# IvanPopov/video-flow-ml

Hardware: AMD Instinct MI355X
Metric: flow-fields/sec @1080p seq5 MOF_sintel (higher is better)
Workload: dtype mixed (per-layer MFMA count, f32 accumulate): {"corr": 1, "update_block.encoder.convf1": 1, "update_block.encoder.convf2": 1, "update_block.gru.convq1.iter": "2a", "update_block.gru.convzr1.iter": 1, "update_block.gru.convzr2.iter": 1, "update_block.mask.0": 1, "update_block.mask.2": 1, "update_bloc

## Files before the change

include/vfml.h:

```cpp
#ifndef VFML_H
#define VFML_H
#include <stddef.h>
#include <stdint.h>

#ifdef __cplusplus
extern "C" {
#endif

#define VFML_ABI_VERSION 25

enum {
  VFML_EPI_NONE = 0,
  VFML_EPI_RELU = 1,
  VFML_EPI_TANH = 2,
  VFML_EPI_SIGMOID = 3,
  VFML_EPI_TANH_RELU = 4,
  VFML_EPI_GRU_ZR = 5,
  VFML_EPI_GRU_Q = 6,
  VFML_EPI_ADD_AUX = 7,
};

enum { VFML_FMT_F32 = 0, VFML_FMT_S16 = 1,
       VFML_FMT_F16 = 2 };

typedef struct vfml_conv_desc {
  const float* in0; int32_t c0; int32_t ld0;
  const float* in1; int32_t c1; int32_t ld1;
  int32_t n, h, w;
  const float* weight;
  const float* bias;
  int32_t cout, kh, kw, stride, pad_h, pad_w;
  float* out; int32_t ldo;
  int32_t epilogue; int32_t split; float out_scale;
  const float* aux0; int32_t ld_aux0;
  const float* aux1; int32_t ld_aux1;
  const float* addend; int32_t ld_addend;
  float* out_t; int32_t ld_out_t;
  int32_t flags;
  double* stats_part;
  float* ksplit_ws;
  const void* proj_hi; const void* proj_lo; int32_t proj_n; int32_t proj_kp; float proj_scale;
  float* proj_out; int32_t ld_proj;
  const float* const* addend_ind;
} vfml_conv_desc;

enum { VFML_STATS_ROWS_F32 = 128, VFML_STATS_ROWS_S16 = 32 };
enum { VFML_CONV_SWAP_CROSS = 1,
       VFML_CONV_MFMA2 = 2, VFML_CONV_MFMA1 = 4, VFML_CONV_MFMA2A = 8,
       VFML_CONV_PER_TAP = 16 };

int vfml_conv2d(const vfml_conv_desc* d, void* stream);

int vfml_conv2d_split(const vfml_conv_desc* d, const void* w_hi, const void* w_lo, int kp, float w_scale,
                      int in_fmt, int out_fmt, int aux_fmt, int k_order, void* stream);
enum { VFML_KORDER_TAP = 0, VFML_KORDER_CBLOCK = 1, VFML_KORDER_CBLOCK64 = 2 };

int vfml_to_s16(const float* src, int64_t rows, int c, int ld_src, float* dst, int ld_dst, float scale, void* stream);

int vfml_split_f16(const float* src, int64_t rows, int k, int ld, float scale, void* hi, void* lo, int kp,
                   void* stream);

int vfml_softmax_rows_s16(const float* x, int64_t rows, int cols, int64_t ld_in, float* out, int64_t ld_out, float scale,
                          void* stream);

int vfml_softmax_rows_f16(const float* x, int64_t rows, int cols, int64_t ld_in, void* out, int64_t ld_out, float scale,
                          void* stream);

int vfml_transpose_to_s16(const float* src, int rows, int c, int ld, float scale, float* dst, int64_t ld_dst, void* stream);

int vfml_add_to_s16(const float* x, int64_t ldx, const float* aux, int64_t ld_aux, float* out, int64_t ld_out, int64_t rows,
                    int c, float scale, void* stream);

int vfml_transpose_split_f16(const float* src, int rows, int c, int ld, float scale, void* hi, void* lo, int kp,
                             void* stream);

int vfml_frames_to_nhwc4(const void* src, int kind, int n, int H, int W,
                         float scale, float shift, float* dst, void* stream);

int64_t vfml_instnorm_workspace_bytes(int n, int hw, int c);
int vfml_instnorm_stats(const float* x, int n, int hw, int c, float eps,
                        float* stats, void* workspace, void* stream);
int vfml_instnorm_apply(const float* x, const float* stats, const float* res,
                        const float* res_stats, int n, int hw, int c, float* out, int out_fmt, void* stream);

int vfml_avgpool2x2(const float* x, int n, int h, int w, int c, float* out, void* stream);

int vfml_corr_lookup(const float* const* pyr, const int32_t* hl, const int32_t* wl,
                     const int32_t* ld, int levels, int radius, int nmaps, int q_per_map,
                     const float* coords, int ld_coords, float* out, int ld_out, int out_fmt, int vol_fmt, int vol_tile,
                     void* stream);
#define VFML_VOL_F16_LEVELS(m) (0x100 | (m))

int vfml_corr_lookup_indirect(const float* const* table, const int32_t* hl, const int32_t* wl, const int32_t* ld,
                              int levels, int radius, int nmaps, int q_per_map, const float* coords, int ld_coords,
                              float* out, int ld_out, int out_fmt, int vol_fmt, int vol_tile, void* stream);
int vfml_corr_lookup_indirect_bidir(const float* const* table, const int32_t* hl, const int32_t* wl, const int32_t* ld,
                                    int levels, int radius, int nmaps, int q_per_map, const float* coords, int ld_coords,
                                    int dir_coords, float* out, int ld_out, int dir_out, int dir_tab, int out_fmt, int vol_fmt,
                                    int vol_tile, void* stream);
int vfml_ptr_table_set(void* table, const void* const* ptrs, int n, void* stream);

int vfml_flow_rows7(const float* flow, int n, int h, int w, float* rows, void* stream);

int vfml_conv3x3_c64(const float* in, int ld_in, int n, int h, int w, const void* w_hi, const void* w_lo, int kp, float w_scale,
                     const float* bias, float* out, int ldo, double* stats_part, void* stream);

int vfml_flow_half(const float* flow, int n, int h, int w, const void* w1_hi, int kp1, float w1_scale, const float* b1,
                   const void* w2_hi, int kp2, float w2_scale, const float* b2, float* out, int ld_out, void* stream);

int vfml_tapsum3x3(const float* t, int ld_t, const float* bias, int n, int h, int w, float* out, int parts, int64_t part_stride,
                   void* stream);
int vfml_tapsum3x3_update(const float* t, int ld_t, const float* bias, int n, int h, int w, int parts, int64_t part_stride,
                          float* coords1, float* flow_a, int ld_a, float* flow_b, int ld_b, int fmt_b, void* stream);

int vfml_coords_update(float* coords1, const float* delta, int n, int h, int w,
                       float* flow_a, int ld_a, float* flow_b, int ld_b, int fmt_b, void* stream);
int vfml_coords_init(float* coords1, int n, int h, int w, void* stream);

int vfml_convex_upsample(const float* coords1, int ch, const float* mask, int ld_mask,
                         int h, int w, float* out, void* stream);

int64_t vfml_instnorm_finalize_workspace_bytes(int chunks, int c);
int vfml_instnorm_finalize(const double* part, int n, int chunks, int c, int hw, float eps, float* stats,
                           void* workspace, int64_t workspace_bytes, void* stream);

int vfml_stem7x7s2_chunks(int h, int w);
int vfml_stem7x7s2(const float* frames, int n, int h, int w, const void* w_hi, const void* w_lo, float w_scale,
                   const float* bias, float* out, double* stats_part, void* stream);

int vfml_flow_lod(const float* flow, int h, int w, float* out, void* stream);

enum { VFML_ENCODE_GAMEDEV = 0, VFML_ENCODE_RG8 = 1, VFML_ENCODE_RGB8 = 2 };
int vfml_flow_encode(const float* flow, int h, int w, int mode, float width, float height, float scale,
                     float clamp, float two_clamp, unsigned char* out, void* stream);

enum { VFML_TAA_SIMPLE = 0, VFML_TAA_BILINEAR = 1, VFML_TAA_BILATERAL = 2 };
enum { VFML_PIX_U8 = 0, VFML_PIX_F32 = 1, VFML_PIX_F64 = 2 };
int vfml_taa_blend(const void* current, int cur_type, const float* flow, const void* history, int hist_type,
                   void* out, int out_type, int h, int w, int mode, double alpha, double sigma_color, void* stream);

int vfml_flow_quality_map(const unsigned char* frame1, const unsigned char* frame2, const float* flow, int fh, int fw,
                          int h, int w, float threshold, unsigned char* out, void* stream);

#define VFML_CORRECT_RECORD 16
size_t vfml_flow_correct_workspace_bytes(int h, int w);
int vfml_flow_correct(const unsigned char* frame1, const unsigned char* frame2, const float* flow, const float* lod,
                      int lh, int lw, int h, int w, const double* twiddles, double good_threshold,
                      double fine_threshold, double region_radius, double template_radius, double search_radius,
                      float* out_flow, int* counts, double* records, int64_t record_capacity, void* workspace,
                      size_t workspace_bytes, void* stream);

enum { VFML_COLORIZE_HSV = 0, VFML_COLORIZE_WHEEL = 1 };
int vfml_flow_colorize(const float* flow, int h, int w, int mode, void* workspace, unsigned char* out, void* stream);

enum { VFML_COMPOSE_SIDE_BY_SIDE = 0, VFML_COMPOSE_STACKED = 1, VFML_COMPOSE_GRID_2X2 = 2 };
enum { VFML_COMPOSE_BGR = 1, VFML_COMPOSE_BOTTOM_UP = 2 };
int vfml_compose_frame(const void* const* tiles, const int* tile_types, int h, int w, int layout, int flags,
                       int64_t row_stride, unsigned char* out, void* stream);

const char* vfml_last_error(void);
int vfml_abi_version(void);

#ifdef __cplusplus
}
#endif
#endif
```

video-flow-ml_amd/vfml/csrc/flow_ops.hip:

```cpp
#include <stdlib.h>
#include "vfml_common.h"

namespace {

constexpr int MAX_LEVELS = 6;
constexpr int MAX_MAPS = 8;
constexpr int MAX_RADIUS = 4;
constexpr int PATCH = 2 * MAX_RADIUS + 2;
#ifndef VFML_LOOKUP_WAVES
#define VFML_LOOKUP_WAVES 4
#endif
constexpr int LOOKUP_WAVES = VFML_LOOKUP_WAVES;
constexpr int FIXED_LEVELS = 4;
static_assert(FIXED_LEVELS == 4, "corr_lookup_fixed_kernel selects among four levels");

struct LookupArgs {
  const float* pyr[MAX_MAPS][MAX_LEVELS];
  const float* const* table;
  int hl[MAX_LEVELS], wl[MAX_LEVELS], ld[MAX_LEVELS];
  int levels, radius, nq, q_per_map;
  const float* coords; int ld_coords;
  float* out; int ld_out;
  int out16;
  int vol16;
  int tws, ths;
  int qw;
  int dir_maps, dir_coords, dir_out;
  int dir_tab;
};

__device__ __forceinline__ void lookup_rows(const LookupArgs& a, int q, int& map, int64_t& crow, int64_t& orow) {
  const int dir = a.dir_maps && map >= a.dir_maps;
  const int64_t qd = q - (dir ? a.dir_maps * a.q_per_map : 0);
  if (dir) map += a.dir_tab - a.dir_maps;
  crow = qd * a.ld_coords + (dir ? a.dir_coords : 0);
  orow = qd * a.ld_out + (dir ? a.dir_out : 0);
}

__device__ __forceinline__ int tiled_at(int y, int x, int w, int tws, int ths) {
  const int tpr = (w + (1 << tws) - 1) >> tws;
  return ((((y >> ths) * tpr + (x >> tws)) << (tws + ths)) + ((y & ((1 << ths) - 1)) << tws) + (x & ((1 << tws) - 1)));
}

__device__ __forceinline__ float bilinear4(float nw, float ne, float sw, float se, float wx0, float fx, float wy0, float fy) {
  float v = ne * (fx * wy0);
  v = __builtin_fmaf(nw, wx0 * wy0, v);
  v = __builtin_fmaf(sw, wx0 * fy, v);
  v = __builtin_fmaf(se, fx * fy, v);
  return v;
}

__global__ __launch_bounds__(64 * LOOKUP_WAVES) void corr_lookup_kernel(const LookupArgs a) {
  __shared__ float patch[LOOKUP_WAVES][MAX_LEVELS][PATCH * PATCH];
  __shared__ float frac[LOOKUP_WAVES][MAX_LEVELS][2];
  const int lane = threadIdx.x & 63;
  const int wv = threadIdx.x >> 6;
  const int q = blockIdx.x * LOOKUP_WAVES + wv;
  const bool live = q < a.nq;
  int map = live ? q / a.q_per_map : 0;
  const int qq = q - map * a.q_per_map;
  const int side = 2 * a.radius + 2;
  const int win = 2 * a.radius + 1;
  const int psz = side * side;
  int64_t crow = 0, orow = 0;
  if (live) lookup_rows(a, q, map, crow, orow);
  if (live) {
    const float cx = a.coords[crow + 0];
    const float cy = a.coords[crow + 1];
    const int total = a.levels * psz;
    const int qrow = (a.tws | a.ths) ? tiled_at(qq / a.qw, qq % a.qw, a.qw, a.tws, a.ths) : qq;
    for (int e = lane; e < total; e += 64) {
      const int l = e / psz;
      const int idx = e - l * psz;
      const int py = idx / side, px = idx - py * side;
      const float inv = 1.0f / (float)(1 << l);
      const float x = cx * inv, y = cy * inv;
      const float fx0 = floorf(x), fy0 = floorf(y);
      const int x0 = (int)fminf(fmaxf(fx0, -65536.f), 65536.f) - a.radius;
      const int y0 = (int)fminf(fmaxf(fy0, -65536.f), 65536.f) - a.radius;
      const int xx = x0 + px, yy = y0 + py;
      float v = 0.f;
      if (xx >= 0 && xx < a.wl[l] && yy >= 0 && yy < a.hl[l])
        v = (a.table ? a.table[map * a.levels + l] : a.pyr[map][l])[(int64_t)qrow * a.ld[l] + tiled_at(yy, xx, a.wl[l], a.tws, a.ths)];
      patch[wv][l][idx] = v;
      if (idx == 0) {
        frac[wv][l][0] = x - fx0;
        frac[wv][l][1] = y - fy0;
      }
    }
  }
  __syncthreads();
  if (!live) return;
  const int nout = a.levels * win * win;
  float* o = a.out + orow;
  const int nwrite = a.out16 ? (nout + 7) & ~7 : nout;
  for (int c = lane; c < nwrite; c += 64) {
    if (c >= nout) {
      _Float16* u = reinterpret_cast<_Float16*>(o + (c & ~7));
      u[c & 7] = (_Float16)0.f;
      u[8 + (c & 7)] = (_Float16)0.f;
      continue;
    }
    const int l = c / (win * win);
    const int rem = c - l * win * win;
    const int i = rem / win, j = rem - i * win;
    const float fx = frac[wv][l][0], fy = frac[wv][l][1];
    const float* p = &patch[wv][l][j * side + i];
    const float wx0 = 1.f - fx, wy0 = 1.f - fy;
    const float v = bilinear4(p[0], p[1], p[side], p[side + 1], wx0, fx, wy0, fy);
    if (a.out16) {
      vfml_h16x2 hh, ll;
      vfml_split2(v, 0.f, hh, ll);
      _Float16* u = reinterpret_cast<_Float16*>(o + (c & ~7));
      u[c & 7] = hh[0];
      u[8 + (c & 7)] = ll[0];
    } else {
      o[c] = v;
    }
  }
}

__device__ __forceinline__ float bilinear4w(float nw, float ne, float sw, float se, float w00, float w10, float w01, float w11) {
  float v = ne * w10;
  v = __builtin_fmaf(nw, w00, v);
  v = __builtin_fmaf(sw, w01, v);
  v = __builtin_fmaf(se, w11, v);
  return v;
}

__device__ __forceinline__ void wave_lds_sync() {
  __builtin_amdgcn_fence(__ATOMIC_RELEASE, "workgroup");
  __builtin_amdgcn_wave_barrier();
  __builtin_amdgcn_fence(__ATOMIC_ACQUIRE, "workgroup");
}

template <int R, bool OUT16, int V16 = 0>
__global__ __launch_bounds__(64 * LOOKUP_WAVES) void corr_lookup_fixed_kernel(const LookupArgs a) {
  constexpr int SIDE = 2 * R + 2, PSZ = SIDE * SIDE, WIN = 2 * R + 1, WW = WIN * WIN;
  constexpr int NOUTPAD = (FIXED_LEVELS * WW + 7) & ~7;
  static_assert(PSZ <= 128 && FIXED_LEVELS * WIN <= 64 && NOUTPAD / 8 <= 64, "one wave: at most two gather passes per level");
  __shared__ float patch[LOOKUP_WAVES][FIXED_LEVELS][PSZ];
  __shared__ __attribute__((aligned(16))) float outs[LOOKUP_WAVES][NOUTPAD];
  const int lane = threadIdx.x & 63;
  const int wv = __builtin_amdgcn_readfirstlane(threadIdx.x >> 6);
  const int q = blockIdx.x * LOOKUP_WAVES + wv;
  if (q >= a.nq) return;
  int map = __builtin_amdgcn_readfirstlane(q / a.q_per_map);
  const int qq = q - map * a.q_per_map;
  const int qrow = __builtin_amdgcn_readfirstlane((a.tws | a.ths) ? tiled_at(qq / a.qw, qq % a.qw, a.qw, a.tws, a.ths) : qq);
  int64_t crow, orow;
  lookup_rows(a, q, map, crow, orow);
  const float cx = a.coords[crow + 0];
  const float cy = a.coords[crow + 1];
  const int pyA = lane / SIDE, pxA = lane - pyA * SIDE;
  const int pyB = (lane + 64) / SIDE, pxB = (lane + 64) - pyB * SIDE;
  const bool inB = lane + 64 < PSZ;
  const float* pl[FIXED_LEVELS];
  if (a.table) {
#pragma unroll
    for (int l = 0; l < FIXED_LEVELS; ++l) pl[l] = a.table[map * a.levels + (l < a.levels ? l : 0)];
  } else {
#pragma unroll
    for (int l = 0; l < FIXED_LEVELS; ++l) pl[l] = a.pyr[map][l < a.levels ? l : 0];
  }
  float va[FIXED_LEVELS], vb[FIXED_LEVELS];
  bool oka[FIXED_LEVELS], okb[FIXED_LEVELS];
#pragma unroll
  for (int l = 0; l < FIXED_LEVELS; ++l) {
    const bool have = l < a.levels;
    const int ll = have ? l : 0;
    const bool v16 = (V16 >> l) & 1;
    const int ES = v16 ? 2 : 4;
    const char* base = reinterpret_cast<const char*>(pl[l]) + (int64_t)qrow * a.ld[ll] * ES;
    const int wl = a.wl[ll], hl = a.hl[ll];
    const float inv = __builtin_bit_cast(float, (127 - l) << 23);
    const float x = cx * inv, y = cy * inv;
    const int x0 = (int)fminf(fmaxf(floorf(x), -65536.f), 65536.f) - R;
    const int y0 = (int)fminf(fmaxf(floorf(y), -65536.f), 65536.f) - R;
    auto texel = [&](int px, int py, bool in, float& out, bool& ok) {
      const int xx = x0 + px, yy = y0 + py;
      ok = have && in && xx >= 0 && xx < wl && yy >= 0 && yy < hl;
      const int at = tiled_at(min(max(yy, 0), hl - 1), min(max(xx, 0), wl - 1), wl, a.tws, a.ths);
      if (v16) out = (float)((const __attribute__((address_space(1))) _Float16*)base)[at];
      else out = ((const __attribute__((address_space(1))) float*)base)[at];
    };
    texel(pxA, pyA, true, va[l], oka[l]);
    if constexpr (PSZ > 64) texel(pxB, pyB, inB, vb[l], okb[l]);
    else { vb[l] = 0.f; okb[l] = false; }
  }
#pragma unroll
  for (int l = 0; l < FIXED_LEVELS; ++l) {
    va[l] = oka[l] ? va[l] : 0.f;
    vb[l] = okb[l] ? vb[l] : 0.f;
  }
#pragma unroll
  for (int l = 0; l < FIXED_LEVELS; ++l) {
    if (l < a.levels) {
      if (PSZ > 64 || lane < PSZ) patch[wv][l][lane] = va[l];
      if constexpr (PSZ > 64) if (inB) patch[wv][l][lane + 64] = vb[l];
    }
  }
  const int nout = a.levels * WW;
  const int nunits = (nout + 7) >> 3;
  if (lane >= 56 && nout + (lane - 56) < nunits * 8) outs[wv][nout + (lane - 56)] = 0.f;
  wave_lds_sync();
  if (lane < a.levels * WIN) {
    const int l = lane / WIN, i = lane - l * WIN;
    const float inv = __builtin_bit_cast(float, (127 - l) << 23);
    const float x = cx * inv, y = cy * inv;
    const float fx = x - floorf(x), fy = y - floorf(y);
    const float wx0 = 1.f - fx, wy0 = 1.f - fy;
    const float w00 = wx0 * wy0, w10 = fx * wy0, w01 = wx0 * fy, w11 = fx * fy;
    const float* p = &patch[wv][l][i];
    float* o = &outs[wv][l * WW + i * WIN];
    float nw = p[0], ne = p[1];
#pragma unroll
    for (int j = 0; j < WIN; ++j) {
      const float sw = p[(j + 1) * SIDE], se = p[(j + 1) * SIDE + 1];
      o[j] = bilinear4w(nw, ne, sw, se, w00, w10, w01, w11);
      nw = sw; ne = se;
    }
  }
  wave_lds_sync();
  if (lane < nunits) {
    float* o = a.out + orow + lane * 8;
    const f32x4 v0 = *reinterpret_cast<const f32x4*>(&outs[wv][lane * 8]);
    const f32x4 v1 = *reinterpret_cast<const f32x4*>(&outs[wv][lane * 8 + 4]);
    if (OUT16) {
      vfml_h16x2 h0, h1, h2, h3, l0, l1, l2, l3;
      vfml_split2(v0[0], v0[1], h0, l0);
      vfml_split2(v0[2], v0[3], h1, l1);
      vfml_split2(v1[0], v1[1], h2, l2);
      vfml_split2(v1[2], v1[3], h3, l3);
      uint4 hv, lv;
      hv.x = __builtin_bit_cast(unsigned, h0); hv.y = __builtin_bit_cast(unsigned, h1);
      hv.z = __builtin_bit_cast(unsigned, h2); hv.w = __builtin_bit_cast(unsigned, h3);
      lv.x = __builtin_bit_cast(unsigned, l0); lv.y = __builtin_bit_cast(unsigned, l1);
      lv.z = __builtin_bit_cast(unsigned, l2); lv.w = __builtin_bit_cast(unsigned, l3);
      *reinterpret_cast<uint4*>(o) = hv;
      *reinterpret_cast<uint4*>(o + 4) = lv;
    } else {
#pragma unroll
      for (int h = 0; h < 2; ++h) {
        const int c = lane * 8 + 4 * h;
        const f32x4 w = h ? v1 : v0;
        if (c + 3 < nout && (((uintptr_t)(o + 4 * h)) & 15u) == 0) {
          *reinterpret_cast<f32x4*>(o + 4 * h) = w;
        } else {
#pragma unroll
          for (int k = 0; k < 4; ++k)
            if (c + k < nout) o[4 * h + k] = w[k];
        }
      }
    }
  }
}

__global__ void coords_init_kernel(f32x4* __restrict__ coords, int h, int w, int64_t total) {
  for (int64_t p = (int64_t)blockIdx.x * blockDim.x + threadIdx.x; p < total; p += (int64_t)gridDim.x * blockDim.x) {
    const int x = (int)(p % w);
    const int y = (int)((p / w) % h);
    f32x4 v = {(float)x, (float)y, (float)x, (float)y};
    coords[p] = v;
  }
}

__global__ void flow_rows7_kernel(const f32x4* __restrict__ flow, int w, int64_t total, char* __restrict__ rows) {
  for (int64_t i = (int64_t)blockIdx.x * blockDim.x + threadIdx.x; i < total * 4; i += (int64_t)gridDim.x * blockDim.x) {
    const int64_t p = i >> 2;
    const int u = (int)(i & 3);
    const int x = (int)(p % w);
    f32x4 t0 = {0.f, 0.f, 0.f, 0.f}, t1 = {0.f, 0.f, 0.f, 0.f};
    const int x0 = x + 2 * u - 3, x1 = x0 + 1;
    if (x0 >= 0 && x0 < w) t0 = flow[p + 2 * u - 3];
    if (u < 3 && x1 >= 0 && x1 < w) t1 = flow[p + 2 * u - 2];
    vfml_h16x2 h[4], l[4];
    vfml_split2(t0[0], t0[1], h[0], l[0]);
    vfml_split2(t0[2], t0[3], h[1], l[1]);
    vfml_split2(t1[0], t1[1], h[2], l[2]);
    vfml_split2(t1[2], t1[3], h[3], l[3]);
    uint4 hv, lv;
    hv.x = __builtin_bit_cast(unsigned, h[0]); hv.y = __builtin_bit_cast(unsigned, h[1]);
    hv.z = __builtin_bit_cast(unsigned, h[2]); hv.w = __builtin_bit_cast(unsigned, h[3]);
    lv.x = __builtin_bit_cast(unsigned, l[0]); lv.y = __builtin_bit_cast(unsigned, l[1]);
    lv.z = __builtin_bit_cast(unsigned, l[2]); lv.w = __builtin_bit_cast(unsigned, l[3]);
    char* o = rows + p * 128 + u * 32;
    *reinterpret_cast<uint4*>(o) = hv;
    *reinterpret_cast<uint4*>(o + 16) = lv;
  }
}

__device__ __forceinline__ void emit_flow(int64_t p, const f32x4 c, int h, int w, float* __restrict__ fa, int lda,
                                          float* __restrict__ fb, int ldb, int b16) {
  const float x = (float)(int)(p % w);
  const float y = (float)(int)((p / w) % h);
  const f32x4 f = {c[0] - x, c[1] - y, c[2] - x, c[3] - y};
  if (fa) *reinterpret_cast<f32x4*>(fa + p * lda) = f;
  if (fb) {
    if (b16) {
      typedef vfml_h16x2 fp16x2_;
      fp16x2_ h0, h1, l0, l1;
      vfml_split2(f[0], f[1], h0, l0);
      vfml_split2(f[2], f[3], h1, l1);
      char* u = reinterpret_cast<char*>(fb + p * ldb) - 16;
      *reinterpret_cast<fp16x2_*>(u + 8) = h0;
      *reinterpret_cast<fp16x2_*>(u + 12) = h1;
      *reinterpret_cast<fp16x2_*>(u + 24) = l0;
      *reinterpret_cast<fp16x2_*>(u + 28) = l1;
    } else {
      *reinterpret_cast<f32x4*>(fb + p * ldb) = f;
    }
  }
}

__global__ void tapsum3x3_kernel(const float* __restrict__ t, int ld, const float* __restrict__ bias, int h, int w,
                                 int64_t total, f32x4* __restrict__ out, int parts, int64_t part_stride,
                                 f32x4* __restrict__ coords, float* __restrict__ fa, int lda, float* __restrict__ fb, int ldb,
                                 int b16) {
  for (int64_t p = (int64_t)blockIdx.x * blockDim.x + threadIdx.x; p < total; p += (int64_t)gridDim.x * blockDim.x) {
    const int x = (int)(p % w), y = (int)((p / w) % h);
    f32x4 s = {0.f, 0.f, 0.f, 0.f};
    if (bias) s = f32x4{bias[0], bias[1], bias[2], bias[3]};
#pragma unroll
    for (int ky = 0; ky < 3; ++ky)
#pragma unroll
      for (int kx = 0; kx < 3; ++kx) {
        const int yy = y + ky - 1, xx = x + kx - 1;
        if (yy >= 0 && yy < h && xx >= 0 && xx < w) {
          const float* q = t + (p + (int64_t)(ky - 1) * w + (kx - 1)) * ld + (ky * 3 + kx) * 4;
          f32x4 v = *reinterpret_cast<const f32x4*>(q);
          for (int k = 1; k < parts; ++k) v = v + *reinterpret_cast<const f32x4*>(q + k * part_stride);
          s = s + v;
        }
      }
    if (out) out[p] = s;
    if (coords) {
      const f32x4 c = coords[p] + s;
      coords[p] = c;
// ... 90 lines not shown
  VFML_REQUIRE(table && ptrs && n >= 1 && n <= MAX_TABLE, "vfml_ptr_table_set: 1..%d pointers", MAX_TABLE);
  PtrTable t;
  for (int i = 0; i < MAX_TABLE; ++i) t.p[i] = i < n ? ptrs[i] : nullptr;
  hipLaunchKernelGGL(ptr_table_kernel, dim3(1), dim3(64), 0, reinterpret_cast<hipStream_t>(stream), t, n,
                     reinterpret_cast<const void**>(table));
  return vfml_check_launch("vfml_ptr_table_set");
}

static int corr_lookup_impl(const float* const* pyr, const float* const* table, const int32_t* hl, const int32_t* wl,
                            const int32_t* ld, int levels, int radius, int nmaps, int q_per_map, const float* coords,
                            int ld_coords, float* out, int ld_out, int out_fmt, int vol_fmt, int vol_tile, void* stream,
                            int dir_maps = 0, int dir_coords = 0, int dir_out = 0, int dir_tab = 0);

extern "C" int vfml_corr_lookup(const float* const* pyr, const int32_t* hl, const int32_t* wl, const int32_t* ld,
                                int levels, int radius, int nmaps, int q_per_map, const float* coords, int ld_coords,
                                float* out, int ld_out, int out_fmt, int vol_fmt, int vol_tile, void* stream) {
  VFML_REQUIRE(pyr, "vfml_corr_lookup: null pointer");
  return corr_lookup_impl(pyr, nullptr, hl, wl, ld, levels, radius, nmaps, q_per_map, coords, ld_coords, out, ld_out, out_fmt,
                          vol_fmt, vol_tile, stream);
}

extern "C" int vfml_corr_lookup_indirect(const float* const* table, const int32_t* hl, const int32_t* wl, const int32_t* ld,
                                         int levels, int radius, int nmaps, int q_per_map, const float* coords,
                                         int ld_coords, float* out, int ld_out, int out_fmt, int vol_fmt, int vol_tile, void* stream) {
  VFML_REQUIRE(table && (reinterpret_cast<uintptr_t>(table) & 7u) == 0, "vfml_corr_lookup_indirect: null / misaligned table");
  return corr_lookup_impl(nullptr, table, hl, wl, ld, levels, radius, nmaps, q_per_map, coords, ld_coords, out, ld_out,
                          out_fmt, vol_fmt, vol_tile, stream);
}

extern "C" int vfml_corr_lookup_indirect_bidir(const float* const* table, const int32_t* hl, const int32_t* wl, const int32_t* ld,
                                               int levels, int radius, int nmaps, int q_per_map, const float* coords,
                                               int ld_coords, int dir_coords, float* out, int ld_out, int dir_out, int dir_tab,
                                               int out_fmt, int vol_fmt, int vol_tile, void* stream) {
  VFML_REQUIRE(table && (reinterpret_cast<uintptr_t>(table) & 7u) == 0, "vfml_corr_lookup_indirect_bidir: null / misaligned table");
  VFML_REQUIRE(nmaps >= 1 && 2 * nmaps <= MAX_MAPS, "vfml_corr_lookup_indirect_bidir: nmaps=%d out of [1,%d]", nmaps, MAX_MAPS / 2);
  VFML_REQUIRE(dir_coords >= 0 && dir_coords + 2 <= ld_coords && dir_out >= 0 && (out_fmt != VFML_FMT_S16 || dir_out % 8 == 0),
               "vfml_corr_lookup_indirect_bidir: dir_coords within a coords row, dir_out >= 0 (a multiple of 8 floats for split rows)");
  VFML_REQUIRE(dir_tab >= nmaps && (dir_tab + nmaps) * levels <= MAX_TABLE,
               "vfml_corr_lookup_indirect_bidir: dir_tab=%d (the second direction's first map in the table) out of range", dir_tab);
  return corr_lookup_impl(nullptr, table, hl, wl, ld, levels, radius, 2 * nmaps, q_per_map, coords, ld_coords, out, ld_out,
                          out_fmt, vol_fmt, vol_tile, stream, nmaps, dir_coords, dir_out, dir_tab);
}

static int corr_lookup_impl(const float* const* pyr, const float* const* table, const int32_t* hl, const int32_t* wl,
                            const int32_t* ld, int levels, int radius, int nmaps, int q_per_map, const float* coords,
                            int ld_coords, float* out, int ld_out, int out_fmt, int vol_fmt, int vol_tile, void* stream,
                            int dir_maps, int dir_coords, int dir_out, int dir_tab) {
  VFML_REQUIRE(nmaps >= 1 && nmaps <= MAX_MAPS && q_per_map > 0, "vfml_corr_lookup: nmaps=%d out of [1,%d] or empty maps", nmaps, MAX_MAPS);
  const int nq = nmaps * q_per_map;
  VFML_REQUIRE(out_fmt == VFML_FMT_F32 || out_fmt == VFML_FMT_S16, "vfml_corr_lookup: bad out_fmt");
  int v16mask = vol_fmt == VFML_FMT_F16 ? 15 : ((vol_fmt & ~15) == VFML_VOL_F16_LEVELS(0) ? (vol_fmt & 15) : (vol_fmt == VFML_FMT_F32 ? 0 : -1));
  if (v16mask > 0 && levels >= 1 && levels <= FIXED_LEVELS) {
    v16mask &= (1 << levels) - 1;
    if (v16mask) v16mask |= 15 & ~((1 << levels) - 1);
  }
  VFML_REQUIRE(v16mask == 0 || ((radius == 3 || radius == 4) && levels <= FIXED_LEVELS &&
                                (v16mask == 15 || v16mask == 14 || v16mask == 12 || v16mask == 8)),
               "vfml_corr_lookup: vol_fmt is VFML_FMT_F32, or (radius 3 / 4, at most %d levels) VFML_FMT_F16 or "
               "VFML_VOL_F16_LEVELS(m) with m = levels 1-3, 2-3 or 3", FIXED_LEVELS);
  VFML_REQUIRE(hl && wl && ld && coords && out, "vfml_corr_lookup: null pointer");
  VFML_REQUIRE(levels >= 1 && levels <= MAX_LEVELS, "vfml_corr_lookup: levels=%d out of [1,%d]", levels, MAX_LEVELS);
  VFML_REQUIRE(radius >= 1 && radius <= MAX_RADIUS, "vfml_corr_lookup: radius=%d out of [1,%d]", radius, MAX_RADIUS);
  VFML_REQUIRE(ld_coords >= 2, "vfml_corr_lookup: bad ld_coords");
  const int nout = levels * (2 * radius + 1) * (2 * radius + 1);
  VFML_REQUIRE(ld_out >= nout, "vfml_corr_lookup: ld_out=%d < %d channels", ld_out, nout);
  if (out_fmt == VFML_FMT_S16)
    VFML_REQUIRE(ld_out % 8 == 0 && ld_out >= ((nout + 7) & ~7) && (reinterpret_cast<uintptr_t>(out) & 31u) == 0,
                 "vfml_corr_lookup: split-row output needs a 32-byte aligned out and ld_out %% 8 == 0");
  LookupArgs a;
  a.out16 = out_fmt == VFML_FMT_S16;
  a.vol16 = v16mask;
  a.table = table;
  for (int m = 0; m < MAX_MAPS; ++m)
    for (int l = 0; l < MAX_LEVELS; ++l) a.pyr[m][l] = nullptr;
  for (int l = 0; l < levels; ++l) {
    VFML_REQUIRE(hl[l] > 0 && wl[l] > 0 && ld[l] >= hl[l] * wl[l], "vfml_corr_lookup: bad level %d", l);
    a.hl[l] = hl[l]; a.wl[l] = wl[l]; a.ld[l] = ld[l];
    for (int m = 0; m < nmaps && pyr; ++m) {
      VFML_REQUIRE(pyr[m * levels + l], "vfml_corr_lookup: null pyramid pointer (map %d, level %d)", m, l);
      a.pyr[m][l] = pyr[m * levels + l];
    }
  }
  for (int l = levels; l < MAX_LEVELS; ++l) a.hl[l] = a.wl[l] = a.ld[l] = 0;
  a.tws = vol_tile & 15; a.ths = (vol_tile >> 4) & 15; a.qw = wl[0];
  VFML_REQUIRE(vol_tile >= 0 && vol_tile < 256 && a.tws <= 6 && a.ths <= 6, "vfml_corr_lookup: vol_tile = tws + 16 * ths with tws, ths <= 6");
  if (vol_tile) {
    VFML_REQUIRE(q_per_map == hl[0] * wl[0], "vfml_corr_lookup: a tiled volume orders its rows by the level-0 grid (q_per_map == hl[0] * wl[0])");
    for (int l = 0; l < levels; ++l)
      VFML_REQUIRE((int64_t)ld[l] >= (int64_t)(((hl[l] - 1) >> a.ths) + 1) * (((wl[l] - 1) >> a.tws) + 1) << (a.tws + a.ths),
                   "vfml_corr_lookup: ld[%d]=%d is less than the whole tiles of a %d x %d level", l, ld[l], wl[l], hl[l]);
  }
  a.levels = levels; a.radius = radius; a.nq = nq; a.q_per_map = q_per_map;
  a.coords = coords; a.ld_coords = ld_coords; a.out = out; a.ld_out = ld_out;
  a.dir_maps = dir_maps; a.dir_coords = dir_coords; a.dir_out = dir_out; a.dir_tab = dir_tab;
  const dim3 grid((nq + LOOKUP_WAVES - 1) / LOOKUP_WAVES), block(64 * LOOKUP_WAVES);
  hipStream_t st = reinterpret_cast<hipStream_t>(stream);
  if (a.vol16) {
    const int m = a.vol16;
#define VFML_LOOKUP16(RR, OO)                                                                                  \
  do {                                                                                                          \
    if (m == 15) hipLaunchKernelGGL((corr_lookup_fixed_kernel<RR, OO, 15>), grid, block, 0, st, a);             \
    else if (m == 14) hipLaunchKernelGGL((corr_lookup_fixed_kernel<RR, OO, 14>), grid, block, 0, st, a);        \
    else if (m == 12) hipLaunchKernelGGL((corr_lookup_fixed_kernel<RR, OO, 12>), grid, block, 0, st, a);        \
    else hipLaunchKernelGGL((corr_lookup_fixed_kernel<RR, OO, 8>), grid, block, 0, st, a);                      \
  } while (0)
    if (radius == 4) {
      if (a.out16) VFML_LOOKUP16(4, true);
      else VFML_LOOKUP16(4, false);
    } else {
      if (a.out16) VFML_LOOKUP16(3, true);
      else VFML_LOOKUP16(3, false);
    }
#undef VFML_LOOKUP16
  } else if (radius == 4 && levels <= FIXED_LEVELS) {
    if (a.out16) hipLaunchKernelGGL((corr_lookup_fixed_kernel<4, true>), grid, block, 0, st, a);
    else hipLaunchKernelGGL((corr_lookup_fixed_kernel<4, false>), grid, block, 0, st, a);
  } else if (radius == 3 && levels <= FIXED_LEVELS) {
    if (a.out16) hipLaunchKernelGGL((corr_lookup_fixed_kernel<3, true>), grid, block, 0, st, a);
    else hipLaunchKernelGGL((corr_lookup_fixed_kernel<3, false>), grid, block, 0, st, a);
  } else {
    hipLaunchKernelGGL(corr_lookup_kernel, grid, block, 0, st, a);
  }
  return vfml_check_launch("vfml_corr_lookup");
}

namespace {
#pragma clang fp contract(off)
__device__ __forceinline__ float np_clip(float x, float lo, float hi) { return x != x ? x : fminf(fmaxf(x, lo), hi); }
__device__ __forceinline__ float np_sqrt(float x) { return (float)sqrt((double)x); }
__device__ __forceinline__ unsigned char np_u8(float v) {
  if (v != v) return 0;
  if (v == INFINITY) return 255;
  if (v == -INFINITY) return 0;
  return (unsigned char)(int)v;
}

struct EncodeArgs {
  const float* flow; unsigned char* out; int64_t n;
  int mode;
  float width, height, scale;
  float clamp, two_clamp;
};

__global__ void flow_encode_kernel(const EncodeArgs a) {
#pragma clang fp contract(off)
  for (int64_t p = (int64_t)blockIdx.x * blockDim.x + threadIdx.x; p < a.n; p += (int64_t)gridDim.x * blockDim.x) {
    float fx = a.flow[2 * p], fy = a.flow[2 * p + 1];
    unsigned char r, g, b;
    if (a.mode == VFML_ENCODE_RGB8) {
      float dx = fx / a.clamp, dy = fy / a.clamp;
      const float len = np_sqrt(dx * dx + dy * dy);
      if (len > 1.0f) {
        dx = dx / len;
        dy = dy / len;
      }
      const float corr = np_sqrt((1.0f - dx * dx) - dy * dy);
      r = np_u8(((np_clip(dx, -1.0f, 1.0f) + 1.0f) / 2.0f) * 255.0f);
      g = np_u8(((np_clip(dy, -1.0f, 1.0f) + 1.0f) / 2.0f) * 255.0f);
      b = np_u8(corr * 255.0f);
    } else {
      if (a.mode == VFML_ENCODE_GAMEDEV) {
        fx = (fx / a.width) * a.scale;
        fy = (fy / a.height) * a.scale;
      }
      const float ex = np_clip((np_clip(fx, -a.clamp, a.clamp) + a.clamp) / a.two_clamp, 0.0f, 1.0f);
      const float ey = np_clip((np_clip(fy, -a.clamp, a.clamp) + a.clamp) / a.two_clamp, 0.0f, 1.0f);
      r = np_u8(ex * 255.0f);
      g = np_u8(ey * 255.0f);
      b = 0;
    }
    a.out[3 * p] = r;
    a.out[3 * p + 1] = g;
    a.out[3 * p + 2] = b;
  }
}
}

extern "C" int vfml_flow_encode(const float* flow, int h, int w, int mode, float width, float height, float scale,
                                float clamp, float two_clamp, unsigned char* out, void* stream) {
  VFML_REQUIRE(flow && out && h > 0 && w > 0, "vfml_flow_encode: bad argument");
// ... 100 lines not shown
```

video-flow-ml_amd/vfml/hip.py:

```python
import ctypes
import os
import subprocess
from ctypes import POINTER, c_char_p, c_double, c_float, c_int, c_int32, c_int64, c_void_p

import torch

_HERE = os.path.dirname(os.path.abspath(__file__))
LIB_PATH = os.environ.get("VFML_LIB") or os.path.join(_HERE, "libvfml_hip.so")
CSRC = os.path.join(_HERE, "csrc")
SOURCES = ["api.hip", "conv_gemm.hip", "conv_gemm_split.hip", "conv_gemm_tapx.hip", "stem.hip", "flow_half.hip", "enc_conv.hip", "norm_pool.hip", "flow_ops.hip", "effects.hip", "correct.hip", "render.hip"]

STATS_ROWS_F32, STATS_ROWS_S16 = 128, 32
EPI_NONE, EPI_RELU, EPI_TANH, EPI_SIGMOID, EPI_TANH_RELU, EPI_GRU_ZR, EPI_GRU_Q, EPI_ADD_AUX = range(8)
FMT_F32, FMT_S16, FMT_F16 = 0, 1, 2


def vol_f16_levels(mask):
    return 0x100 | mask


def _vol_mask(vol_fmt, levels):
    return (15 if vol_fmt == FMT_F16 else (vol_fmt & 15 if vol_fmt & 0x100 else 0)) & ((1 << levels) - 1)

KORDER_TAP, KORDER_CBLOCK, KORDER_CBLOCK64 = 0, 1, 2
CONV_SWAP_CROSS, CONV_MFMA2, CONV_MFMA1, CONV_MFMA2A, CONV_PER_TAP = 1, 2, 4, 8, 16


class ConvDesc(ctypes.Structure):
    _fields_ = [
        ("in0", c_void_p), ("c0", c_int32), ("ld0", c_int32),
        ("in1", c_void_p), ("c1", c_int32), ("ld1", c_int32),
        ("n", c_int32), ("h", c_int32), ("w", c_int32),
        ("weight", c_void_p), ("bias", c_void_p),
        ("cout", c_int32), ("kh", c_int32), ("kw", c_int32), ("stride", c_int32),
        ("pad_h", c_int32), ("pad_w", c_int32),
        ("out", c_void_p), ("ldo", c_int32),
        ("epilogue", c_int32), ("split", c_int32), ("out_scale", c_float),
        ("aux0", c_void_p), ("ld_aux0", c_int32),
        ("aux1", c_void_p), ("ld_aux1", c_int32),
        ("addend", c_void_p), ("ld_addend", c_int32),
        ("out_t", c_void_p), ("ld_out_t", c_int32),
        ("flags", c_int32),
        ("stats_part", c_void_p),
        ("ksplit_ws", c_void_p),
        ("proj_hi", c_void_p), ("proj_lo", c_void_p), ("proj_n", c_int32), ("proj_kp", c_int32), ("proj_scale", c_float),
        ("proj_out", c_void_p), ("ld_proj", c_int32),
        ("addend_ind", c_void_p),
    ]


COMMON_FLAGS = ["-fno-slp-vectorize"]
EXTRA_FLAGS = {}


def build(force=False, verbose=False):
    srcs = [os.path.join(CSRC, s) for s in SOURCES]
    hdrs = [os.path.join(CSRC, "vfml_common.h"), os.path.join(CSRC, "conv_split_common.h"),
            os.path.join(_HERE, "..", "..", "include", "vfml.h")]
    deps = srcs + hdrs
    if not force and os.path.exists(LIB_PATH) and all(
            os.path.getmtime(LIB_PATH) >= os.path.getmtime(d) for d in deps):
        return LIB_PATH
    objdir = os.path.join(CSRC, "_obj")
    os.makedirs(objdir, exist_ok=True)
    newest_hdr = max(os.path.getmtime(h) for h in hdrs)
    jobs = []
    for src in srcs:
        obj = os.path.join(objdir, os.path.basename(src) + ".o")
        if force or not os.path.exists(obj) or os.path.getmtime(obj) < max(os.path.getmtime(src), newest_hdr):
            cmd = ["hipcc", "--offload-arch=gfx950", "-O3", "-std=c++17", "-fPIC"] + COMMON_FLAGS + EXTRA_FLAGS.get(os.path.basename(src), []) + [
                "-c", src, "-o", obj]
            if verbose:
                print(" ".join(cmd))
            jobs.append((cmd, subprocess.Popen(cmd)))
    for cmd, p in jobs:
        if p.wait() != 0:
            raise subprocess.CalledProcessError(p.returncode, cmd)
    cmd = ["hipcc", "--offload-arch=gfx950", "-fPIC", "-shared", "-o", LIB_PATH] + [
        os.path.join(objdir, os.path.basename(src) + ".o") for src in srcs]
    if verbose:
        print(" ".join(cmd))
    subprocess.run(cmd, check=True)
    return LIB_PATH


_lib = None


def lib():
    global _lib
    if _lib is not None:
        return _lib
    if not os.path.exists(LIB_PATH):
        raise RuntimeError(
            f"vfml HIP extension not built: {LIB_PATH} is missing. Run `python -c 'import __graft_entry__ as g; "
            f"g.build()'` (needs hipcc). There is no CPU fallback for the flow engine.")
    L = ctypes.CDLL(LIB_PATH)
    L.vfml_last_error.restype = c_char_p
    L.vfml_abi_version.restype = c_int
    L.vfml_conv2d.argtypes = [POINTER(ConvDesc), c_void_p]
    L.vfml_conv2d_split.argtypes = [POINTER(ConvDesc), c_void_p, c_void_p, c_int, c_float, c_int, c_int, c_int, c_int,
                                    c_void_p]
    L.vfml_to_s16.argtypes = [c_void_p, c_int64, c_int, c_int, c_void_p, c_int, c_float, c_void_p]
    L.vfml_softmax_rows_s16.argtypes = [c_void_p, c_int64, c_int, c_int64, c_void_p, c_int64, c_float, c_void_p]
    L.vfml_transpose_split_f16.argtypes = [c_void_p, c_int, c_int, c_int, c_float, c_void_p, c_void_p, c_int, c_void_p]
# ... 647 lines not shown
```

Baseline: 45.29.

## Add lane-parallel correlation lookup kernel spreading 16 lanes per pyramid level

Adds a new corr_lookup_lanes_kernel for tiled correlation volumes. It gives each pyramid level 16 lanes of a wave, uses a 2D/3D grid ordered by tile, and shares row offsets through ds_bpermute so each lane issues a few independent gathers straight from global memory. The old shared-memory mix and store tail is factored into a reusable helper. The new path becomes the default when the volume is tiled and has 4 levels with radius 3 or 4, and an UNROLLED flag keeps the old kernel reachable. It makes LookupArgs larger and adds complex index arithmetic that could be wrong at boundaries.

```diff
diff --git a/include/vfml.h b/include/vfml.h
--- a/include/vfml.h
+++ b/include/vfml.h
@@ -90,6 +90,7 @@
                      const float* coords, int ld_coords, float* out, int ld_out, int out_fmt, int vol_fmt, int vol_tile,
                      void* stream);
 #define VFML_VOL_F16_LEVELS(m) (0x100 | (m))
+#define VFML_VOL_TILE_UNROLLED 0x100
 
 int vfml_corr_lookup_indirect(const float* const* table, const int32_t* hl, const int32_t* wl, const int32_t* ld,
                               int levels, int radius, int nmaps, int q_per_map, const float* coords, int ld_coords,
diff --git a/video-flow-ml_amd/vfml/csrc/flow_ops.hip b/video-flow-ml_amd/vfml/csrc/flow_ops.hip
--- a/video-flow-ml_amd/vfml/csrc/flow_ops.hip
+++ b/video-flow-ml_amd/vfml/csrc/flow_ops.hip
@@ -27,6 +27,8 @@
   int qw;
   int dir_maps, dir_coords, dir_out;
   int dir_tab;
+  int4 lv[FIXED_LEVELS];
+  const float* mcoords[MAX_MAPS]; float* mout[MAX_MAPS]; int mtab[MAX_MAPS];
 };
 
 __device__ __forceinline__ void lookup_rows(const LookupArgs& a, int q, int& map, int64_t& crow, int64_t& orow) {
@@ -134,6 +136,65 @@
   __builtin_amdgcn_fence(__ATOMIC_ACQUIRE, "workgroup");
 }
 
+template <int R, bool OUT16>
+__device__ __forceinline__ void lookup_mix_store(float* patch, float* outs, int lane, int levels, float cx, float cy, float* out) {
+  constexpr int SIDE = 2 * R + 2, PSZ = SIDE * SIDE, WIN = 2 * R + 1, WW = WIN * WIN;
+  const int nout = levels * WW;
+  const int nunits = (nout + 7) >> 3;
+  if (lane >= 56 && nout + (lane - 56) < nunits * 8) outs[nout + (lane - 56)] = 0.f;
+  wave_lds_sync();
+  if (lane < levels * WIN) {
+    const int l = lane / WIN, i = lane - l * WIN;
+    const float inv = __builtin_bit_cast(float, (127 - l) << 23);
+    const float x = cx * inv, y = cy * inv;
+    const float fx = x - floorf(x), fy = y - floorf(y);
+    const float wx0 = 1.f - fx, wy0 = 1.f - fy;
+    const float w00 = wx0 * wy0, w10 = fx * wy0, w01 = wx0 * fy, w11 = fx * fy;
+    const float* p = &patch[l * PSZ + i];
+    float* o = &outs[l * WW + i * WIN];
+    float nw = p[0], ne = p[1];
+#pragma unroll
+    for (int j = 0; j < WIN; ++j) {
+      const float sw = p[(j + 1) * SIDE], se = p[(j + 1) * SIDE + 1];
+      o[j] = bilinear4w(nw, ne, sw, se, w00, w10, w01, w11);
+      nw = sw; ne = se;
+    }
+  }
+  wave_lds_sync();
+  if (lane < nunits) {
+    float* o = out + lane * 8;
+    const f32x4 v0 = *reinterpret_cast<const f32x4*>(&outs[lane * 8]);
+    const f32x4 v1 = *reinterpret_cast<const f32x4*>(&outs[lane * 8 + 4]);
+    if (OUT16) {
+      vfml_h16x2 h0, h1, h2, h3, l0, l1, l2, l3;
+      vfml_split2(v0[0], v0[1], h0, l0);
+      vfml_split2(v0[2], v0[3], h1, l1);
+      vfml_split2(v1[0], v1[1], h2, l2);
+      vfml_split2(v1[2], v1[3], h3, l3);
+      uint4 hv, lv;
+      hv.x = __builtin_bit_cast(unsigned, h0); hv.y = __builtin_bit_cast(unsigned, h1);
+      hv.z = __builtin_bit_cast(unsigned, h2); hv.w = __builtin_bit_cast(unsigned, h3);
+      lv.x = __builtin_bit_cast(unsigned, l0); lv.y = __builtin_bit_cast(unsigned, l1);
+      lv.z = __builtin_bit_cast(unsigned, l2); lv.w = __builtin_bit_cast(unsigned, l3);
+      *reinterpret_cast<uint4*>(o) = hv;
+      *reinterpret_cast<uint4*>(o + 4) = lv;
+    } else {
+#pragma unroll
+      for (int h = 0; h < 2; ++h) {
+        const int c = lane * 8 + 4 * h;
+        const f32x4 w = h ? v1 : v0;
+        if (c + 3 < nout && (((uintptr_t)(o + 4 * h)) & 15u) == 0) {
+          *reinterpret_cast<f32x4*>(o + 4 * h) = w;
+        } else {
+#pragma unroll
+          for (int k = 0; k < 4; ++k)
+            if (c + k < nout) o[4 * h + k] = w[k];
+        }
+      }
+    }
+  }
+}
+
 template <int R, bool OUT16, int V16 = 0>
 __global__ __launch_bounds__(64 * LOOKUP_WAVES) void corr_lookup_fixed_kernel(const LookupArgs a) {
   constexpr int SIDE = 2 * R + 2, PSZ = SIDE * SIDE, WIN = 2 * R + 1, WW = WIN * WIN;
@@ -200,60 +261,104 @@
       if constexpr (PSZ > 64) if (inB) patch[wv][l][lane + 64] = vb[l];
     }
   }
-  const int nout = a.levels * WW;
-  const int nunits = (nout + 7) >> 3;
-  if (lane >= 56 && nout + (lane - 56) < nunits * 8) outs[wv][nout + (lane - 56)] = 0.f;
-  wave_lds_sync();
-  if (lane < a.levels * WIN) {
-    const int l = lane / WIN, i = lane - l * WIN;
-    const float inv = __builtin_bit_cast(float, (127 - l) << 23);
-    const float x = cx * inv, y = cy * inv;
-    const float fx = x - floorf(x), fy = y - floorf(y);
-    const float wx0 = 1.f - fx, wy0 = 1.f - fy;
-    const float w00 = wx0 * wy0, w10 = fx * wy0, w01 = wx0 * fy, w11 = fx * fy;
-    const float* p = &patch[wv][l][i];
-    float* o = &outs[wv][l * WW + i * WIN];
-    float nw = p[0], ne = p[1];
-#pragma unroll
-    for (int j = 0; j < WIN; ++j) {
-      const float sw = p[(j + 1) * SIDE], se = p[(j + 1) * SIDE + 1];
-      o[j] = bilinear4w(nw, ne, sw, se, w00, w10, w01, w11);
-      nw = sw; ne = se;
-    }
-  }
-  wave_lds_sync();
-  if (lane < nunits) {
-    float* o = a.out + orow + lane * 8;
-    const f32x4 v0 = *reinterpret_cast<const f32x4*>(&outs[wv][lane * 8]);
-    const f32x4 v1 = *reinterpret_cast<const f32x4*>(&outs[wv][lane * 8 + 4]);
-    if (OUT16) {
-      vfml_h16x2 h0, h1, h2, h3, l0, l1, l2, l3;
-      vfml_split2(v0[0], v0[1], h0, l0);
-      vfml_split2(v0[2], v0[3], h1, l1);
-      vfml_split2(v1[0], v1[1], h2, l2);
-      vfml_split2(v1[2], v1[3], h3, l3);
-      uint4 hv, lv;
-      hv.x = __builtin_bit_cast(unsigned, h0); hv.y = __builtin_bit_cast(unsigned, h1);
-      hv.z = __builtin_bit_cast(unsigned, h2); hv.w = __builtin_bit_cast(unsigned, h3);
-      lv.x = __builtin_bit_cast(unsigned, l0); lv.y = __builtin_bit_cast(unsigned, l1);
-      lv.z = __builtin_bit_cast(unsigned, l2); lv.w = __builtin_bit_cast(unsigned, l3);
-      *reinterpret_cast<uint4*>(o) = hv;
-      *reinterpret_cast<uint4*>(o + 4) = lv;
-    } else {
-#pragma unroll
-      for (int h = 0; h < 2; ++h) {
-        const int c = lane * 8 + 4 * h;
-        const f32x4 w = h ? v1 : v0;
-        if (c + 3 < nout && (((uintptr_t)(o + 4 * h)) & 15u) == 0) {
-          *reinterpret_cast<f32x4*>(o + 4 * h) = w;
-        } else {
-#pragma unroll
-          for (int k = 0; k < 4; ++k)
-            if (c + k < nout) o[4 * h + k] = w[k];
-        }
-      }
-    }
-  }
+  lookup_mix_store<R, OUT16>(&patch[wv][0][0], outs[wv], lane, a.levels, cx, cy, a.out + orow);
+}
+
+template <int R, bool OUT16, int V16 = 0>
+__global__ __launch_bounds__(64 * LOOKUP_WAVES) void corr_lookup_lanes_kernel(const LookupArgs a) {
+  typedef const __attribute__((address_space(1))) unsigned* gptr_u32;
+  typedef const __attribute__((address_space(1))) uint64_t* gptr_u64;
+  constexpr int SIDE = 2 * R + 2, PSZ = SIDE * SIDE, WIN = 2 * R + 1, WW = WIN * WIN;
+  constexpr int NOUTPAD = (FIXED_LEVELS * WW + 7) & ~7;
+  constexpr int NA = SIDE / 2;
+  constexpr int NB = SIDE - 8;
+  constexpr int RB = NB ? 16 / NB : 1;
+  constexpr int NPB = NB ? (SIDE + RB - 1) / RB : 0;
+  static_assert(SIDE >= 8 && (NB == 0 || NB == 2) && FIXED_LEVELS * 16 == 64 && FIXED_LEVELS * WIN <= 64, "sixteen lanes per level");
+  __shared__ float patch[LOOKUP_WAVES][FIXED_LEVELS][PSZ];
+  __shared__ __attribute__((aligned(16))) float outs[LOOKUP_WAVES][NOUTPAD];
+  const int lane = threadIdx.x & 63;
+  const int wv = __builtin_amdgcn_readfirstlane(threadIdx.x >> 6);
+  const int sh = a.tws + a.ths;
+  const int u = blockIdx.x * LOOKUP_WAVES + wv;
+  const int qx = ((u >> sh) << a.tws) + (u & ((1 << a.tws) - 1));
+  const int qy = (blockIdx.y << a.ths) + ((u >> a.tws) & ((1 << a.ths) - 1));
+  if (qx >= a.qw || qy >= a.lv[0].y) return;
+  const unsigned qrow = ((blockIdx.y * a.lv[0].w) << sh) + u;
+  const int map = blockIdx.z, qq = qy * a.qw + qx;
+  const float* cq = a.mcoords[map] + (int64_t)qq * a.ld_coords;
+  const float cx = cq[0], cy = cq[1];
+  const int l = lane >> 4, c = lane & 15;
+  const int4 lv = a.lv[l];
+  const int wl = lv.x, hl = lv.y, tpr = lv.w;
+  const bool v16 = (V16 >> l) & 1;
+  const int es = v16 ? 1 : 2;
+  const uint64_t ptrs = a.table ? reinterpret_cast<uint64_t>(a.table + a.mtab[map] * FIXED_LEVELS)
+                                : reinterpret_cast<uint64_t>(__builtin_amdgcn_kernarg_segment_ptr()) + offsetof(LookupArgs, pyr) + map * sizeof(a.pyr[0]);
+  uint64_t base = ((gptr_u64)ptrs)[l] + (((uint64_t)qrow * (unsigned)lv.z) << es);
+  unsigned odd = 0;
+  if (V16) { odd = v16 ? (unsigned)base & 2u : 0u; base -= odd; }
+  const float inv = __builtin_bit_cast(float, (127 - l) << 23);
+  const float x = cx * inv, y = cy * inv;
+  const int x0 = (int)fminf(fmaxf(floorf(x), -65536.f), 65536.f) - R;
+  const int y0 = (int)fminf(fmaxf(floorf(y), -65536.f), 65536.f) - R;
+  const int mw = (1 << a.tws) - 1, mh = (1 << a.ths) - 1;
+  const int yy = y0 + c;
+  const int yc = min(max(yy, 0), hl - 1);
+  const unsigned yoff = ((__umul24(yc >> a.ths, tpr) << sh) + ((yc & mh) << a.tws)) << es;
+  const unsigned rows_in = (unsigned)(__builtin_amdgcn_ballot_w64((unsigned)yy < (unsigned)hl) >> (lane & 48));
+  auto column = [&](int px, uint64_t& p, unsigned& in, unsigned& half) {
+    const int xx = x0 + px;
+    const int xc = min(max(xx, 0), wl - 1);
+    unsigned xoff = ((((xc >> a.tws) << sh) + (xc & mw)) << es) + odd;
+    half = 0;
+    if (V16) { half = (xoff & 2u) << 3; xoff &= ~3u; }
+    p = base + xoff;
+    in = (unsigned)xx < (unsigned)wl ? rows_in : 0u;
+  };
+  constexpr int NT = NA + NPB;
+  const int rowA = c >> 3, rowB = NB ? c / (NB ? NB : 1) : 0;
+  const int rowL = NB ? rowB + (rowB + RB * (NPB - 1) < SIDE ? RB * (NPB - 1) : RB * (NPB - 2)) : 0;
+  uint64_t pA, pB = 0;
+  unsigned inA, inB = 0, halfA, halfB = 0;
+  column(c & 7, pA, inA, halfA);
+  if constexpr (NB > 0) column(8 + (c & (NB - 1)), pB, inB, halfB);
+  inA >>= rowA;
+  unsigned off[NT], okm[NT], v[NT];
+  const int srcA = ((lane & 48) + rowA) * 4, srcB = ((lane & 48) + rowB) * 4, srcL = ((lane & 48) + rowL) * 4;
+#pragma unroll
+  for (int k = 0; k < NA; ++k) {
+    off[k] = (unsigned)__builtin_amdgcn_ds_bpermute(srcA + 8 * k, (int)yoff);
+    okm[k] = (unsigned)((int)(inA << (31 - 2 * k)) >> 31);
+  }
+#pragma unroll
+  for (int k = 0; k < NPB; ++k) {
+    const bool last = k == NPB - 1 && NPB * RB > SIDE;
+    off[NA + k] = (unsigned)__builtin_amdgcn_ds_bpermute(last ? srcL : srcB + 4 * RB * k, (int)yoff);
+    okm[NA + k] = (unsigned)((int)((inB >> (last ? rowL : rowB + RB * k)) << 31) >> 31);
+  }
+#pragma unroll
+  for (int k = 0; k < NT; ++k) v[k] = *(gptr_u32)((k < NA ? pA : pB) + off[k]);
+  const unsigned m16 = v16 ? ~0u : 0u;
+  float f[NT];
+#pragma unroll
+  for (int k = 0; k < NT; ++k) {
+    unsigned t = v[k];
+    if (V16) {
+      const float h = (float)__builtin_bit_cast(_Float16, (unsigned short)(t >> (k < NA ? halfA : halfB)));
+      t = (__builtin_bit_cast(unsigned, h) & m16) | (t & ~m16);
+    }
+    f[k] = __builtin_bit_cast(float, t & okm[k]);
+  }
+  float* pl = &patch[wv][l][0];
+#pragma unroll
+  for (int k = 0; k < NA; ++k) pl[(rowA + 2 * k) * SIDE + (c & 7)] = f[k];
+#pragma unroll
+  for (int k = 0; k < NPB; ++k) {
+    const bool last = k == NPB - 1 && NPB * RB > SIDE;
+    pl[(last ? rowL : rowB + RB * k) * SIDE + 8 + (c & (NB ? NB - 1 : 0))] = f[NA + k];
+  }
+  lookup_mix_store<R, OUT16>(&patch[wv][0][0], outs[wv], lane, FIXED_LEVELS, cx, cy, a.mout[map] + (int64_t)qq * a.ld_out);
 }
 
 __global__ void coords_init_kernel(f32x4* __restrict__ coords, int h, int w, int64_t total) {
@@ -510,6 +615,8 @@
     }
   }
   for (int l = levels; l < MAX_LEVELS; ++l) a.hl[l] = a.wl[l] = a.ld[l] = 0;
+  const bool unrolled = vol_tile >= 0 && (vol_tile & VFML_VOL_TILE_UNROLLED);
+  if (unrolled) vol_tile &= ~VFML_VOL_TILE_UNROLLED;
   a.tws = vol_tile & 15; a.ths = (vol_tile >> 4) & 15; a.qw = wl[0];
   VFML_REQUIRE(vol_tile >= 0 && vol_tile < 256 && a.tws <= 6 && a.ths <= 6, "vfml_corr_lookup: vol_tile = tws + 16 * ths with tws, ths <= 6");
   if (vol_tile) {
@@ -523,7 +630,36 @@
   a.dir_maps = dir_maps; a.dir_coords = dir_coords; a.dir_out = dir_out; a.dir_tab = dir_tab;
   const dim3 grid((nq + LOOKUP_WAVES - 1) / LOOKUP_WAVES), block(64 * LOOKUP_WAVES);
   hipStream_t st = reinterpret_cast<hipStream_t>(stream);
-  if (a.vol16) {
+  for (int l = 0; l < FIXED_LEVELS; ++l)
+    a.lv[l] = l < levels ? make_int4(wl[l], hl[l], ld[l], ((wl[l] - 1) >> a.tws) + 1) : make_int4(0, 0, 0, 0);
+  for (int m = 0; m < MAX_MAPS; ++m) {
+    const int dir = dir_maps && m >= dir_maps, mm = m < nmaps ? m - (dir ? dir_maps : 0) : 0;
+    a.mcoords[m] = coords + (int64_t)mm * q_per_map * ld_coords + (dir ? dir_coords : 0);
+    a.mout[m] = out + (int64_t)mm * q_per_map * ld_out + (dir ? dir_out : 0);
+    a.mtab[m] = m + (dir ? dir_tab - dir_maps : 0);
+  }
+  bool lanes = vol_tile && !unrolled && a.tws >= 1 && levels == FIXED_LEVELS && (radius == 3 || radius == 4);
+  for (int l = 0; l < levels && lanes; ++l) lanes = hl[l] < (1 << 24) && wl[l] < (1 << 24) && ld[l] < (1 << 28);
+  if (lanes) {
+    const dim3 tgrid(((a.lv[0].w << (a.tws + a.ths)) + LOOKUP_WAVES - 1) / LOOKUP_WAVES, ((hl[0] - 1) >> a.ths) + 1, nmaps);
+    VFML_REQUIRE(tgrid.y <= 65535, "vfml_corr_lookup: %d tile rows of queries", (int)tgrid.y);
+#define VFML_LOOKUP_LANES(RR, OO)                                                                               \
+  do {                                                                                                          \
+    if (a.vol16 == 0) hipLaunchKernelGGL((corr_lookup_lanes_kernel<RR, OO, 0>), tgrid, block, 0, st, a);        \
+    else if (a.vol16 == 15) hipLaunchKernelGGL((corr_lookup_lanes_kernel<RR, OO, 15>), tgrid, block, 0, st, a); \
+    else if (a.vol16 == 14) hipLaunchKernelGGL((corr_lookup_lanes_kernel<RR, OO, 14>), tgrid, block, 0, st, a); \
+    else if (a.vol16 == 12) hipLaunchKernelGGL((corr_lookup_lanes_kernel<RR, OO, 12>), tgrid, block, 0, st, a); \
+    else hipLaunchKernelGGL((corr_lookup_lanes_kernel<RR, OO, 8>), tgrid, block, 0, st, a);                     \
+  } while (0)
+    if (radius == 4) {
+      if (a.out16) VFML_LOOKUP_LANES(4, true);
+      else VFML_LOOKUP_LANES(4, false);
+    } else {
+      if (a.out16) VFML_LOOKUP_LANES(3, true);
+      else VFML_LOOKUP_LANES(3, false);
+    }
+#undef VFML_LOOKUP_LANES
+  } else if (a.vol16) {
     const int m = a.vol16;
 #define VFML_LOOKUP16(RR, OO)                                                                                  \
   do {                                                                                                          \
diff --git a/video-flow-ml_amd/vfml/hip.py b/video-flow-ml_amd/vfml/hip.py
--- a/video-flow-ml_amd/vfml/hip.py
+++ b/video-flow-ml_amd/vfml/hip.py
@@ -21,6 +21,8 @@
 
 def _vol_mask(vol_fmt, levels):
     return (15 if vol_fmt == FMT_F16 else (vol_fmt & 15 if vol_fmt & 0x100 else 0)) & ((1 << levels) - 1)
+
+VOL_TILE_UNROLLED = 0x100
 
 KORDER_TAP, KORDER_CBLOCK, KORDER_CBLOCK64 = 0, 1, 2
 CONV_SWAP_CROSS, CONV_MFMA2, CONV_MFMA1, CONV_MFMA2A, CONV_PER_TAP = 1, 2, 4, 8, 16
```

Result: no change. 45.63 (median of 6 runs) (+0.8%).
